# george-gca/sr-pytorch-lightning

Measured on AMD Instinct MI355X. Metric: SR training throughput, LR patches/s (48x48 LR x4, fwd+bwd+Adam), higher is better.
Workload: dtype bf16; 1 GPU; edsr_baseline x4, 48x48 LR patches, batch 256/GPU, train step (L1 + Adam); global_batch=256, parallelism=dp1, hip_graph=full

## Files before the change

### sr-pytorch-lightning_amd/csrc/hr_tail.hip

```cpp
#include "srk_common.h"

namespace {

SRK_DEV void sub_of(int a, int d, int& i, int& s) {
  const int ap = a + d;
  i = ap & 1;
  s = (ap - i) >> 1;
}

struct Wts {
  const float* wt; const float* bt; const float* wu; const float* bu;
  int O, C, Ci;
};

SRK_DEV float sum16(float v) {
  v += __shfl_xor(v, 8, 64);
  v += __shfl_xor(v, 4, 64);
  v += __shfl_xor(v, 2, 64);
  v += __shfl_xor(v, 1, 64);
  return v;
}

SRK_DEV float collapse_w(const Wts& p, int sub, int o, int a, int b, int ci, int dy0, int dy1, int dx0, int dx1, int fy, int fx) {
  float acc = 0.f;
// ... 216 lines not shown
  const bool shared_line = phase == 0 ? H == 1 : W == 1;
  if (shared_line && blockIdx.y == 1) return;
  extern __shared__ __attribute__((aligned(16))) char smem_raw[];
  const size_t gplane = (size_t)H2 * W2;
  const float* const g = a.g + (size_t)n * O * gplane;
  for (int rep = 0; rep < (shared_line ? 2 : 1); ++rep) {
  const EdgeGeo e = edge_geo(2 * phase + (shared_line ? rep : (int)blockIdx.y), H, W);
  float* const Gl = reinterpret_cast<float*>(smem_raw);
  float* const Wl = Gl + (size_t)2 * O * (e.len + 4);
  __syncthreads();
  for (int i0 = threadIdx.x; i0 < 2 * O * (e.len + 4); i0 += 256 * 4) {
    float v[4];
#pragma unroll
    for (int u = 0; u < 4; ++u) {
      const int i = i0 + 256 * u;
      const int kk = i / (e.len + 4), s = i % (e.len + 4) - 2, o = kk >> 1, q = kk & 1;
      v[u] = 0.f;
      if (i < 2 * O * (e.len + 4) && s >= 0 && s < e.len)
        v[u] = e.row ? g[(size_t)o * gplane + (size_t)e.fix_hr * W2 + 2 * s + q] : g[(size_t)o * gplane + (size_t)(2 * s + q) * W2 + e.fix_hr];
    }
#pragma unroll
    for (int u = 0; u < 4; ++u)
      if (i0 + 256 * u < 2 * O * (e.len + 4)) Gl[i0 + 256 * u] = v[u];
  }
  stage_copy256(Wl, a.wedge + (size_t)e.ty * 2 * O * Ci * 5, 2 * O * Ci * 5);
  __syncthreads();
  const int nch = (Ci + 7) >> 3;
  const bool vec = (Ci & 7) == 0 && (a.dx_pitch & 7) == 0;
  for (int idx = threadIdx.x + 256 * blockIdx.z; idx < e.len * nch; idx += 256 * gridDim.z) {
    const int c8 = idx % nch, s = idx / nch;
    float corr[8];
#pragma unroll
    for (int k = 0; k < 8; ++k) corr[k] = 0.f;
    for (int kk = 0; kk < 2 * O; ++kk) {
      const float* const gl = Gl + (size_t)kk * (e.len + 4) + s + 2;
      float gv[5];
#pragma unroll
      for (int tt = 0; tt < 5; ++tt) gv[tt] = gl[2 - tt];
#pragma unroll
      for (int k = 0; k < 8; ++k) {
        const int ci = c8 * 8 + k;
        if (ci < Ci) {
          const float* const w = Wl + ((size_t)kk * Ci + ci) * 5;
#pragma unroll
          for (int tt = 0; tt < 5; ++tt) corr[k] += w[tt] * gv[tt];
        }
      }
    }
    if (!e.row && (s == 0 || s == e.len - 1)) {
      for (int ca = 0; ca < 2; ++ca) {
        if (!(ca ? s == e.len - 1 : s == 0)) continue;
        const int cb = e.ty == 2 ? 0 : 1, c = ca * 2 + cb;
        const size_t at = (size_t)(ca ? H2 - 1 : 0) * W2 + e.fix_hr;
        for (int o = 0; o < O; ++o) {
          const float gc = g[(size_t)o * gplane + at];
#pragma unroll
          for (int k = 0; k < 8; ++k)
            if (c8 * 8 + k < Ci) corr[k] -= a.wcor[((size_t)c * O + o) * Ci + c8 * 8 + k] * gc;
        }
      }
    }
    const int yy = e.row ? e.fix_lr : s, xx = e.row ? s : e.fix_lr;
    typename Tr::elem* const d = reinterpret_cast<typename Tr::elem*>(a.dx) + ((size_t)(n * H + yy) * W + xx) * a.dx_pitch + c8 * 8;
    if (vec) {
      const i32x4 raw = *reinterpret_cast<const i32x4*>(d);
      const int w4[4] = {raw.x, raw.y, raw.z, raw.w};
      int o4[4];
#pragma unroll
      for (int k = 0; k < 4; ++k) {
        float f0, f1;
        unpack2<DT>((uint32_t)w4[k], f0, f1);
        o4[k] = (int)pack2<DT>(f0 - corr[2 * k], f1 - corr[2 * k + 1]);
      }
      *reinterpret_cast<i32x4*>(d) = i32x4{o4[0], o4[1], o4[2], o4[3]};
    } else {
#pragma unroll
      for (int k = 0; k < 8; ++k)
        if (c8 * 8 + k < Ci) d[k] = Tr::from_f32(Tr::to_f32(d[k]) - corr[k]);
    }
  }
  }
}

constexpr int EW_MAXLEN = 512;
template <int DT>
__global__ __launch_bounds__(256) void hrtail_edge_bwd_w_kernel(const srk_hrtail_args a, int nchunks, int ew_chunk) {
  const int H = a.H, W = a.W, O = a.O, Ci = a.Ci, H2 = 2 * H, W2 = 2 * W;
  const int ty = blockIdx.y, chunk = blockIdx.x;
  const int n0 = chunk * ew_chunk, n1 = min(a.N, n0 + ew_chunk);
  const int ncombo = ty < 4 ? 2 * O * 5 : O;
  const size_t gplane = (size_t)H2 * W2;
  float* const dst = a.scratch + ((size_t)ty * nchunks + chunk) * (size_t)(2 * MAXO * 5) * (Ci + 1);
  extern __shared__ __attribute__((aligned(16))) char smem_raw[];
  float* const Xl = reinterpret_cast<float*>(smem_raw);
  if (ty >= 4) {
    if (blockIdx.z != 0) return;
    const int c = ty - 4, ca = c >> 1, cbb = c & 1;
    const int Py = ca ? H2 - 1 : 0, Px = cbb ? W2 - 1 : 0, yy = ca ? H - 1 : 0, xx = cbb ? W - 1 : 0;
    for (int item = threadIdx.x; item < ncombo * (Ci + 1); item += 256) {
      const int ci = item % (Ci + 1), o = item / (Ci + 1);
      float acc = 0.f;
      for (int n = n0; n < n1; ++n) {
        const float gv = a.g[((size_t)n * O + o) * gplane + (size_t)Py * W2 + Px];
        const float xv = ci < Ci ? ld_act<DT>(a.x, ((size_t)(n * H + yy) * W + xx) * a.x_pitch + ci) : 1.f;
        acc += gv * xv;
      }
      dst[item] = acc;
    }
    return;
  }
  const bool rowedge = ty < 2;
  const int len = rowedge ? W : H;
  float* const Gl = Xl + (size_t)(len + 4) * Ci;
  constexpr int MAXIT = (2 * MAXO * 5 * 65 + 255) / 256;
  const int nitems = ncombo * (Ci + 1);
  const int ipb = (nitems + gridDim.z - 1) / gridDim.z, item0 = blockIdx.z * ipb, item1 = min(nitems, item0 + ipb);
  float acc[MAXIT];
#pragma unroll
  for (int k = 0; k < MAXIT; ++k) acc[k] = 0.f;
  for (int n = n0; n < n1; ++n) {
    __syncthreads();
    stage_line<DT>(a, edge_geo(ty, H, W), n, Xl, Ci);
    for (int i = threadIdx.x; i < 2 * O * len; i += 256) {
      const int kk = i / len, s = i % len, o = kk >> 1, q = kk & 1;
      const float* const g = a.g + ((size_t)n * O + o) * gplane;
      Gl[i] = rowedge ? g[(size_t)(ty == 0 ? 0 : H2 - 1) * W2 + 2 * s + q] : g[(size_t)(2 * s + q) * W2 + (ty == 2 ? 0 : W2 - 1)];
    }
    __syncthreads();
#pragma unroll
    for (int k = 0; k < MAXIT; ++k) {
      const int item = item0 + threadIdx.x + k * 256;
      if (item >= item1) break;
      const int ci = item % (Ci + 1), cb = item / (Ci + 1), tt = cb % 5, kk = cb / 5;
      const float* const gr = Gl + kk * len;
      float t0 = 0.f, t1 = 0.f, t2 = 0.f, t3 = 0.f;
      int p = 0;
      if (ci < Ci) {
        const float* const xr = Xl + (size_t)tt * Ci + ci;
        for (; p + 3 < len; p += 4) {
          t0 += gr[p] * xr[(size_t)p * Ci]; t1 += gr[p + 1] * xr[(size_t)(p + 1) * Ci];
          t2 += gr[p + 2] * xr[(size_t)(p + 2) * Ci]; t3 += gr[p + 3] * xr[(size_t)(p + 3) * Ci];
        }
        for (; p < len; ++p) t0 += gr[p] * xr[(size_t)p * Ci];
      } else if (tt == 2) {
        for (; p + 3 < len; p += 4) { t0 += gr[p]; t1 += gr[p + 1]; t2 += gr[p + 2]; t3 += gr[p + 3]; }
        for (; p < len; ++p) t0 += gr[p];
      }
      acc[k] += (t0 + t1) + (t2 + t3);
    }
  }
#pragma unroll
  for (int k = 0; k < MAXIT; ++k) {
    const int item = item0 + threadIdx.x + k * 256;
    if (item < item1) dst[item] = acc[k];
  }
}

__global__ __launch_bounds__(256) void hrtail_edge_reduce_kernel(const srk_hrtail_args a, int nchunks) {
  const int O = a.O, Ci = a.Ci;
  const int per = 2 * MAXO * 5 * (Ci + 1);
  const int t = blockIdx.x * 256 + threadIdx.x;
  const int n_edge = 4 * 2 * O * 5 * (Ci + 1), n_cor = 4 * O * (Ci + 1);
  if (t >= n_edge + n_cor) return;
  int ty, item;
  if (t < n_edge) { ty = t / (2 * O * 5 * (Ci + 1)); item = t % (2 * O * 5 * (Ci + 1)); }
  else { const int u = t - n_edge; ty = 4 + u / (O * (Ci + 1)); item = u % (O * (Ci + 1)); }
// ... 63 lines not shown
      }
    }
    acc = wave_total(acc);
    if (lane == 0) a.dwt[t] = acc;
    return;
  }
  int t = blockIdx.x * 256 + threadIdx.x;
  if (t < n_wu) {
    const int e = t % 9, ci = (t / 9) % Ci, cu = t / (9 * Ci), c = cu >> 2, i = (cu >> 1) & 1, j = cu & 1;
    const int ey = e / 3 - 1, ex = e % 3 - 1;
    float acc = 0.f;
    for (int pa = 0; pa < 2; ++pa)
      for (int dy = -1; dy <= 1; ++dy) {
        int ii, sy; sub_of(pa, dy, ii, sy);
        if (ii != i) continue;
        for (int pb = 0; pb < 2; ++pb)
          for (int dx = -1; dx <= 1; ++dx) {
            int jj, sx; sub_of(pb, dx, jj, sx);
            if (jj != j) continue;
            for (int o = 0; o < O; ++o)
              acc += a.wt[((size_t)o * C + c) * 9 + (dy + 1) * 3 + dx + 1] * g_w(q, o, pa, pb, dy, dx, ci, sy + ey, sx + ex);
          }
      }
    a.dwu[t] = acc;
    return;
  }
  t -= n_wu;
  if (t < n_bu) {
    if (!a.dbu) return;
    const int cu = t, c = cu >> 2, i = (cu >> 1) & 1, j = cu & 1;
    float acc = 0.f;
    for (int pa = 0; pa < 2; ++pa)
      for (int dy = -1; dy <= 1; ++dy) {
        int ii, sy; sub_of(pa, dy, ii, sy);
        if (ii != i) continue;
        for (int pb = 0; pb < 2; ++pb)
          for (int dx = -1; dx <= 1; ++dx) {
            int jj, sx; sub_of(pb, dx, jj, sx);
            if (jj != j) continue;
            for (int o = 0; o < O; ++o) acc += a.wt[((size_t)o * C + c) * 9 + (dy + 1) * 3 + dx + 1] * g_b(q, o, pa, pb, dy, dx);
          }
      }
    a.dbu[cu] = acc;
    return;
  }
  t -= n_bu;
  if (t < n_bt && a.dbt) a.dbt[t] = a.r0[t * 4] + a.r0[t * 4 + 1] + a.r0[t * 4 + 2] + a.r0[t * 4 + 3];
}

int check_common(const srk_hrtail_args* a, const char* who) {
  SRK_CHECK_ARG(a, "%s: null argument", who);
  SRK_CHECK_ARG(a->O >= 1 && a->O <= MAXO && a->C >= 1 && a->Ci >= 1, "%s: O=%d (1..%d) C=%d Ci=%d", who, a->O, MAXO, a->C, a->Ci);
  return 0;
}
int check_act(const srk_hrtail_args* a, const char* who) {
  SRK_CHECK_ARG(a->N > 0 && a->H > 0 && a->W > 0, "%s: bad dims N=%d H=%d W=%d", who, a->N, a->H, a->W);
  SRK_CHECK_ARG(a->dtype == SRK_BF16 || a->dtype == SRK_F16, "%s: 16-bit activations only", who);
  SRK_CHECK_ARG((long long)a->N * a->O * 4 * a->H * a->W < (1ll << 31), "%s: output too large", who);
  return 0;
}

}

extern "C" int srk_hrtail_collapse(const srk_hrtail_args* a, srk_stream_t stream) {
  if (int rc = check_common(a, "srk_hrtail_collapse")) return rc;
  SRK_CHECK_ARG(a->wt && a->wu && a->weff && a->beff && a->wedge && a->bedge && a->wcor && a->bcor, "srk_hrtail_collapse: null pointer");
  const int total = 4 * a->O * a->Ci * 25 + 4 * 2 * a->O * a->Ci * 5 + 4 * a->O * a->Ci + 16 * a->O;
  hipLaunchKernelGGL(hrtail_collapse_kernel, dim3((unsigned)((total + 15) / 16)), dim3(256), 0, reinterpret_cast<hipStream_t>(stream), *a);
  SRK_LAUNCH_CHECK();
  return 0;
}

static unsigned edge_split(int N) {
  const int z = (512 + 2 * N - 1) / (2 * N);
  return (unsigned)(z < 1 ? 1 : (z > 8 ? 8 : z));
}

template <typename K> static int edge_lds_attr(K kernel, const char* who) {
  const hipError_t e = hipFuncSetAttribute(reinterpret_cast<const void*>(kernel), hipFuncAttributeMaxDynamicSharedMemorySize, 160 * 1024);
  if (e != hipSuccess) { srk_set_error("%s: cannot reserve LDS: %s", who, hipGetErrorString(e)); return (int)e; }
  return 0;
}

extern "C" int srk_hrtail_edge_fwd(const srk_hrtail_args* a, srk_stream_t stream) {
  if (int rc = check_common(a, "srk_hrtail_edge_fwd")) return rc;
  if (int rc = check_act(a, "srk_hrtail_edge_fwd")) return rc;
  SRK_CHECK_ARG(a->x && a->out && a->wedge && a->bedge && a->wcor && a->bcor, "srk_hrtail_edge_fwd: null pointer");
  const int len = a->H > a->W ? a->H : a->W;
  const size_t lds = ((size_t)(len + 4) * (a->Ci + 1) + (size_t)2 * a->O * a->Ci * 5) * 4;
  SRK_CHECK_ARG(lds <= 160 * 1024, "srk_hrtail_edge_fwd: edge of %d pixels x %d channels does not fit the LDS", len, a->Ci);
  static const int rc0 = edge_lds_attr(&hrtail_edge_fwd_kernel<SRK_BF16>, "srk_hrtail_edge_fwd");
  static const int rc1 = edge_lds_attr(&hrtail_edge_fwd_kernel<SRK_F16>, "srk_hrtail_edge_fwd");
  if (rc0 || rc1) return rc0 ? rc0 : rc1;
  hipStream_t st = reinterpret_cast<hipStream_t>(stream);
  for (int phase = 0; phase < 2; ++phase) {
    if (a->dtype == SRK_BF16) hipLaunchKernelGGL(hrtail_edge_fwd_kernel<SRK_BF16>, dim3((unsigned)a->N, 2, edge_split(a->N)), dim3(256), lds, st, *a, phase);
    else hipLaunchKernelGGL(hrtail_edge_fwd_kernel<SRK_F16>, dim3((unsigned)a->N, 2, edge_split(a->N)), dim3(256), lds, st, *a, phase);
    SRK_LAUNCH_CHECK();
  }
  return 0;
}

extern "C" int srk_hrtail_edge_bwd_x(const srk_hrtail_args* a, srk_stream_t stream) {
  if (int rc = check_common(a, "srk_hrtail_edge_bwd_x")) return rc;
  if (int rc = check_act(a, "srk_hrtail_edge_bwd_x")) return rc;
  SRK_CHECK_ARG(a->g && a->dx && a->wedge && a->wcor, "srk_hrtail_edge_bwd_x: null pointer");
  const int len = a->H > a->W ? a->H : a->W;
  const size_t lds = ((size_t)2 * a->O * (len + 4) + (size_t)2 * a->O * a->Ci * 5) * 4;
  SRK_CHECK_ARG(lds <= 160 * 1024, "srk_hrtail_edge_bwd_x: edge of %d pixels does not fit the LDS", len);
  static const int rc0 = edge_lds_attr(&hrtail_edge_bwd_x_kernel<SRK_BF16>, "srk_hrtail_edge_bwd_x");
  static const int rc1 = edge_lds_attr(&hrtail_edge_bwd_x_kernel<SRK_F16>, "srk_hrtail_edge_bwd_x");
  if (rc0 || rc1) return rc0 ? rc0 : rc1;
  hipStream_t st = reinterpret_cast<hipStream_t>(stream);
  for (int phase = 0; phase < 2; ++phase) {
    if (a->dtype == SRK_BF16) hipLaunchKernelGGL(hrtail_edge_bwd_x_kernel<SRK_BF16>, dim3((unsigned)a->N, 2, edge_split(a->N)), dim3(256), lds, st, *a, phase);
    else hipLaunchKernelGGL(hrtail_edge_bwd_x_kernel<SRK_F16>, dim3((unsigned)a->N, 2, edge_split(a->N)), dim3(256), lds, st, *a, phase);
    SRK_LAUNCH_CHECK();
  }
  return 0;
}

static int ew_chunk_of(int N) { return N <= 64 ? 1 : (N + 63) / 64; }

extern "C" long long srk_hrtail_scratch_floats(int N, int Ci) {
  const int ewc = ew_chunk_of(N);
  const long long nchunks = (N + ewc - 1) / ewc;
  return 8 * nchunks * (long long)(2 * MAXO * 5) * (Ci + 1);
}

extern "C" int srk_hrtail_edge_bwd_w(const srk_hrtail_args* a, srk_stream_t stream) {
  if (int rc = check_common(a, "srk_hrtail_edge_bwd_w")) return rc;
  if (int rc = check_act(a, "srk_hrtail_edge_bwd_w")) return rc;
  SRK_CHECK_ARG(a->x && a->g && a->scratch && a->eedge && a->e0 && a->ecor && a->k0, "srk_hrtail_edge_bwd_w: null pointer");
  const int ewc = ew_chunk_of(a->N);
  const int nchunks = (a->N + ewc - 1) / ewc;
  const unsigned nz = nchunks * 8 >= 512 ? 2 : (nchunks * 8 >= 256 ? 4 : 8);
  const int len = a->H > a->W ? a->H : a->W;
  SRK_CHECK_ARG(a->Ci <= 64 && len <= EW_MAXLEN, "srk_hrtail_edge_bwd_w: Ci=%d (<= 64) edge length %d (<= %d)", a->Ci, len, EW_MAXLEN);
  const size_t lds = ((size_t)(len + 4) * a->Ci + (size_t)2 * a->O * len) * 4;
  hipStream_t st = reinterpret_cast<hipStream_t>(stream);
  static const hipError_t attr0 = hipFuncSetAttribute(reinterpret_cast<const void*>(&hrtail_edge_bwd_w_kernel<SRK_BF16>), hipFuncAttributeMaxDynamicSharedMemorySize, 160 * 1024);
  static const hipError_t attr1 = hipFuncSetAttribute(reinterpret_cast<const void*>(&hrtail_edge_bwd_w_kernel<SRK_F16>), hipFuncAttributeMaxDynamicSharedMemorySize, 160 * 1024);
  if (attr0 != hipSuccess || attr1 != hipSuccess) { srk_set_error("srk_hrtail_edge_bwd_w: cannot reserve LDS"); return (int)(attr0 != hipSuccess ? attr0 : attr1); }
  if (a->dtype == SRK_BF16) hipLaunchKernelGGL(hrtail_edge_bwd_w_kernel<SRK_BF16>, dim3((unsigned)nchunks, 8, nz), dim3(256), lds, st, *a, nchunks, ewc);
  else hipLaunchKernelGGL(hrtail_edge_bwd_w_kernel<SRK_F16>, dim3((unsigned)nchunks, 8, nz), dim3(256), lds, st, *a, nchunks, ewc);
  SRK_LAUNCH_CHECK();
  const int total = (4 * 2 * a->O * 5 + 4 * a->O) * (a->Ci + 1);
  hipLaunchKernelGGL(hrtail_edge_reduce_kernel, dim3((unsigned)((total + 255) / 256)), dim3(256), 0, st, *a, nchunks);
  SRK_LAUNCH_CHECK();
  return 0;
}

extern "C" int srk_hrtail_expand(const srk_hrtail_args* a, srk_stream_t stream) {
  if (int rc = check_common(a, "srk_hrtail_expand")) return rc;
  SRK_CHECK_ARG(a->wt && a->wu && a->r && a->r0 && a->eedge && a->e0 && a->ecor && a->k0 && a->dwt && a->dwu, "srk_hrtail_expand: null pointer");
  const int per_thread = 4 * a->C * a->Ci * 9 + 4 * a->C + a->O, per_wave = a->O * a->C * 9;
  const int nblocks = (per_thread + 255) / 256 + (per_wave + 3) / 4;
  hipLaunchKernelGGL(hrtail_expand_kernel, dim3((unsigned)nblocks), dim3(256), 0, reinterpret_cast<hipStream_t>(stream), *a);
  SRK_LAUNCH_CHECK();
  return 0;
}
```

### sr-pytorch-lightning_amd/csrc/conv_lk.hip

```cpp
#include <stdlib.h>
#include <type_traits>
#include "srk_common.h"

#ifndef SRK_LK5_STAMPS
#define SRK_LK5_STAMPS 0
#endif

namespace {

template <int DT, int CPP, int NRB, int K>
__global__ __launch_bounds__(256) void lk_conv_kernel(const srk_conv_args a, int tilesX, int tilesY, unsigned x_bytes, unsigned w_bytes) {
  typedef DTraits<DT> Tr;
  constexpr int PXB = CPP * 16;
  constexpr int ROWS = 32 * NRB;
  extern __shared__ __attribute__((aligned(16))) char smem[];
  constexpr int XT = 16 + K - 1, XTP = (XT + 1) & ~1;
  constexpr int xs_bytes = XT * XTP * PXB;
  constexpr int slab = K * CPP * ROWS * 16;
  char* const Xs = smem;
  char* const Wr = smem + ((xs_bytes + 1023) & ~1023);

  const int tid = threadIdx.x, lane = tid & 63;
  const int wave = __builtin_amdgcn_readfirstlane(tid >> 6);
  const int r = lane & 31, h = lane >> 5;
// ... 976 lines not shown
      if (lane < 8)
        dma16_hidden(xrsrc, (rok && (unsigned)(x0 + p1) < (unsigned)W) ? (unsigned)(base + c1) : 0x80000000u, (unsigned)__builtin_amdgcn_readfirstlane((int)(dst + 1024)));
    };
    asm volatile("s_waitcnt vmcnt(0) lgkmcnt(0)\n\ts_barrier" ::: "memory");
    dma_row(wave);
    dma_row(4 + wave);
    dma_row(8 + wave);
#if SRK_LK5_STAMPS
    unsigned long long* const stamp = (blockIdx.x == 0 && tid == 0 && u == blockIdx.x) ? reinterpret_cast<unsigned long long*>(const_cast<float*>(a.post_add)) : nullptr;
#define SRK_LSTAMP(i) do { if (stamp && s < 24) stamp[s * 8 + (i)] = __builtin_amdgcn_s_memtime(); } while (0)
#else
#define SRK_LSTAMP(i) do { } while (0)
#endif
    f32x16 accp[2];
    int gyp = 0;
    uint32_t P[4][4];
    auto epi_cvt = [&](int k) {
#pragma unroll
      for (int d = 0; d < 4; ++d) P[k][d] = pack2<DT>(accp[k >> 1][8 * (k & 1) + 2 * d], accp[k >> 1][8 * (k & 1) + 2 * d + 1]);
    };
    auto epi_store = [&](int j) {
      const int qi = r & 3, gxq = x0 + (r & ~3);
      const bool ok = gyp < ye && gxq + j < W;
      const unsigned off = (unsigned)((((n * H + gyp) * W + gxq + j) * a.out_pitch + a.out_coff + 32 * h + 8 * qi) * 2);
      const u32x4_t ov = {P[j][0], P[j][1], P[j][2], P[j][3]};
      __builtin_amdgcn_raw_buffer_store_b128(ov, orsrc, ok ? off : 0x80000000u, 0, SRK_AUX_WT);
    };
    auto step = [&](int s, auto epi_tag) {
      constexpr bool EPI = decltype(epi_tag)::value;
      SRK_LSTAMP(0);
      if (!EPI) asm volatile("s_waitcnt vmcnt(0)" ::: "memory");
      else if (s == 1) asm volatile("s_waitcnt vmcnt(2)" ::: "memory");
      else if (s == 2) asm volatile("s_waitcnt vmcnt(6)" ::: "memory");
      else asm volatile("s_waitcnt vmcnt(10)" ::: "memory");
      SRK_LSTAMP(1);
      asm volatile("s_waitcnt lgkmcnt(0)\n\ts_barrier" ::: "memory");
      SRK_LSTAMP(2);
      dma_row(4 * s + 12 + wave);
      const int q0 = 4 * s + wave;
      const char* rowp[5];
#pragma unroll
      for (int kh = 0; kh < 5; ++kh) rowp[kh] = smem + ((q0 + kh) % RING) * ROWB + r * 32 + h * 16;
      f32x16 acc[2];
#pragma unroll
      for (int e = 0; e < 16; ++e) { acc[0][e] = 0.f; acc[1][e] = 0.f; }
      constexpr int PF = 6;
      i32x4 bf[PF];
      auto bfrag = [&](int t) { return lds_read16(rowp[t / 5] + (t % 5) * 32); };
#pragma unroll
      for (int t = 0; t < PF; ++t) bf[t] = bfrag(t);
#pragma unroll
      for (int t = 0; t < 25; t += 2) {
        const i32x4 b0 = bf[t % PF], b1 = bf[(t + 1) % PF];
        if (t + PF < 25) bf[t % PF] = bfrag(t + PF);
        if (t + 1 + PF < 25) bf[(t + 1) % PF] = bfrag(t + 1 + PF);
        if (EPI) {
          if (t >= 2 && t < 10) epi_cvt((t - 2) >> 1);
          else if (t == 10) quad_transpose8_dpp(P[0][0], P[1][0], P[2][0], P[3][0], P[0][1], P[1][1], P[2][1], P[3][1]);
          else if (t == 12) quad_transpose8_dpp(P[0][2], P[1][2], P[2][2], P[3][2], P[0][3], P[1][3], P[2][3], P[3][3]);
          else if (t >= 14 && t < 22) epi_store((t - 14) >> 1);
        }
        acc[0] = Tr::mma(A[t][0], b0, acc[0]);
        if (t + 1 < 25) acc[0] = Tr::mma(A[t + 1][0], b1, acc[0]);
        acc[1] = Tr::mma(A[t][1], b0, acc[1]);
        if (t + 1 < 25) acc[1] = Tr::mma(A[t + 1][1], b1, acc[1]);
        __builtin_amdgcn_sched_barrier(0);
      }
      SRK_LSTAMP(3);
      accp[0] = acc[0]; accp[1] = acc[1];
      gyp = ys + q0;
    };
    step(0, std::false_type{});
#pragma unroll 1
    for (int s = 1; s < steps; ++s) step(s, std::true_type{});
#pragma unroll
    for (int k = 0; k < 4; ++k) epi_cvt(k);
    quad_transpose8_dpp(P[0][0], P[1][0], P[2][0], P[3][0], P[0][1], P[1][1], P[2][1], P[3][1]);
    quad_transpose8_dpp(P[0][2], P[1][2], P[2][2], P[3][2], P[0][3], P[1][3], P[2][3], P[3][3]);
#pragma unroll
    for (int j = 0; j < 4; ++j) epi_store(j);
  }
}

SRK_DEV void lk5_pair(int t, int& fyA, int& fxA, int& fyB, int& fxB, bool& hasB) {
  hasB = true;
  if (t < 5) { fyA = -2; fxA = t - 2; fyB = -1; fxB = t - 2; }
  else if (t < 10) { fyA = 0; fxA = t - 7; fyB = 1; fxB = t - 7; }
  else if (t == 10) { fyA = 2; fxA = -2; fyB = 2; fxB = 2; }
  else { fyA = 2; fxA = t - 12; fyB = 2; fxB = t - 12; hasB = false; }
}

template <int DT>
__global__ __launch_bounds__(256) void lk5_wgrad_kernel(const srk_wgrad_args a, int tilesX, int tilesY, int tq, int trem,
                                                        unsigned x_bytes, unsigned dy_bytes) {
  typedef DTraits<DT> Tr;
  constexpr int XB = 16 * 16 * 128, DP = 20, DB = 13 * 1024, BUF = XB + DB;
  extern __shared__ __attribute__((aligned(16))) char smem[];
  const int tid = threadIdx.x, lane = tid & 63;
  const int wave = __builtin_amdgcn_readfirstlane(tid >> 6);
  const int slot = blockIdx.x;
  const int H = a.H, W = a.W;
  const int t0 = slot * tq + min(slot, trem), nt = tq + (slot < trem ? 1 : 0);
  const i32x4 xrs = make_rsrc4(a.x, x_bytes), drs = make_rsrc4(a.dy, dy_bytes);
  const unsigned lds0 = lds_addr_of(smem);

  int xconst[8], xyx[8];
#pragma unroll
  for (int k = 0; k < 8; ++k) {
    const int i = tid + 256 * k, sl = i & 7, p = i >> 3, iy = p >> 4, ix = p & 15, c = sl ^ swz(ix);
    xconst[k] = ((iy * W + ix) * a.x_pitch + a.x_coff + c * 8) * 2;
    xyx[k] = iy | (ix << 8);
  }
  int dconst[4], dyx[4];
#pragma unroll
  for (int j = 0; j < 4; ++j) {
    const int i = tid + 256 * j, c = i & 1, pp = i >> 1, iy = pp / DP, ix = pp - iy * DP;
    dconst[j] = (((iy - 2) * W + (ix - 2)) * a.dy_pitch + a.dy_coff + c * 8) * 2;
    dyx[j] = i < 2 * DP * DP ? (((iy - 2) & 0xffff) | ((ix - 2) << 16)) : (int)0x7fff7fff;
  }
  auto dma_tile = [&](int tile, int b) {
    int pt = tile;
    const int tX = pt % tilesX;
    pt /= tilesX;
    const int tY = pt % tilesY;
    const int n = pt / tilesY;
    const int y0 = tY * 16, x0 = tX * 16;
    const int xbase = ((n * H + y0) * W + x0) * a.x_pitch * 2, dbase = ((n * H + y0) * W + x0) * a.dy_pitch * 2;
#pragma unroll
    for (int k = 0; k < 8; ++k) {
      const bool ok = y0 + (xyx[k] & 255) < H && x0 + (xyx[k] >> 8) < W;
      dma16_hidden(xrs, ok ? (unsigned)(xbase + xconst[k]) : 0x80000000u,
                   (unsigned)__builtin_amdgcn_readfirstlane((int)(lds0 + b * BUF + ((k * 256 + wave * 64) << 4))));
    }
#pragma unroll
    for (int j = 0; j < 4; ++j) {
      if (j * 256 + wave * 64 >= 2 * DP * DP) continue;
      const int gy = y0 + (int)(short)(dyx[j] & 0xffff), gx = x0 + (dyx[j] >> 16);
      const bool ok = (unsigned)gy < (unsigned)H && (unsigned)gx < (unsigned)W;
      dma16_hidden(drs, ok ? (unsigned)(dbase + dconst[j]) : 0x80000000u,
                   (unsigned)__builtin_amdgcn_readfirstlane((int)(lds0 + b * BUF + XB + ((j * 256 + wave * 64) << 4))));
    }
  };

  const int rb = wave & 1, half = wave >> 1;
  f32x16 acc[7];
#pragma unroll
  for (int j = 0; j < 7; ++j)
#pragma unroll
    for (int e = 0; e < 16; ++e) acc[j][e] = 0.f;
  int aoff[2], boff[7][2];
#pragma unroll
  for (int rd = 0; rd < 2; ++rd) aoff[rd] = tr_lane_off(0, rd, rb, lane);
  {
    const int G = lane >> 4, q = (lane & 15) >> 2, pq = lane & 3;
#pragma unroll
    for (int j = 0; j < 7; ++j) {
      int fyA, fxA, fyB, fxB; bool hasB;
      lk5_pair(half * 7 + j, fyA, fxA, fyB, fxB, hasB);
      const int fy = (G & 1) ? fyB : fyA, fx = (G & 1) ? fxB : fxA;
#pragma unroll
      for (int rd = 0; rd < 2; ++rd) {
        const int col = 8 * (G >> 1) + 4 * rd + q;
        boff[j][rd] = ((2 - fy) * DP + (col - fx + 2)) * 32 + pq * 8;
      }
    }
  }
  const bool do_bias = a.dbp != nullptr && wave == 2;
  float dbz = 0.f;

  const int pieces_of = 8 + (wave == 0 ? 4 : 3);
  if (nt > 0) dma_tile(t0, 0);
  if (nt > 1) dma_tile(t0 + 1, 1);
#if SRK_LK5_STAMPS
  unsigned long long* const wstamp = (blockIdx.x == 0 && tid == 0 && a.dbp) ? reinterpret_cast<unsigned long long*>(a.dbp) + (size_t)a.nslabs * 8 : nullptr;
#define SRK_WSTAMP(i) do { if (wstamp && it < 24) wstamp[it * 8 + (i)] = __builtin_amdgcn_s_memtime(); } while (0)
#else
#define SRK_WSTAMP(i) do { } while (0)
#endif
  for (int it = 0; it < nt; ++it) {
    SRK_WSTAMP(0);
    const char* const X = smem + (it % 3) * BUF;
    const char* const D = X + XB;
    if (it + 1 < nt) { if (pieces_of == 12) asm volatile("s_waitcnt vmcnt(12)" ::: "memory"); else asm volatile("s_waitcnt vmcnt(11)" ::: "memory"); }
    else asm volatile("s_waitcnt vmcnt(0)" ::: "memory");
    SRK_WSTAMP(1);
    asm volatile("s_waitcnt lgkmcnt(0)\n\ts_barrier" ::: "memory");
    SRK_WSTAMP(2);
    if (it + 2 < nt) dma_tile(t0 + it + 2, (it + 2) % 3);
    SRK_WSTAMP(3);
    i32x4 afn, bfn[7];
    auto fetch = [&](int y) {
      afn = tr_read2(X + y * 2048 + aoff[0], X + y * 2048 + aoff[1]);
#pragma unroll
      for (int j = 0; j < 7; ++j) bfn[j] = tr_read2(D + y * (DP * 32) + boff[j][0], D + y * (DP * 32) + boff[j][1]);
    };
    fetch(0);
#pragma unroll 2
    for (int y = 0; y < 16; ++y) {
      const i32x4 af = afn;
      i32x4 bf[7];
#pragma unroll
      for (int j = 0; j < 7; ++j) bf[j] = bfn[j];
      if (y + 1 < 16) fetch(y + 1);
      if (do_bias) {
        const int qw[4] = {bf[0].x, bf[0].y, bf[0].z, bf[0].w};
#pragma unroll
        for (int e = 0; e < 4; ++e) {
          float f0, f1;
          unpack2<DT>((uint32_t)qw[e], f0, f1);
          dbz += f0 + f1;
        }
      }
#pragma unroll
      for (int j = 0; j < 7; ++j) acc[j] = Tr::mma(af, bf[j], acc[j]);
    }
    SRK_WSTAMP(4);
  }

  if (do_bias) {
    dbz += __shfl_xor(dbz, 32, 64);
    if (lane < 16) a.dbp[(size_t)slot * 16 + lane] = dbz;
  }
  {
    const int hq = lane >> 5, n = lane & 31, co = n & 15;
    float* const sl = a.dwp + (size_t)slot * (25 * 64 * 16);
#pragma unroll
    for (int j = 0; j < 7; ++j) {
      int fyA, fxA, fyB, fxB; bool hasB;
      lk5_pair(half * 7 + j, fyA, fxA, fyB, fxB, hasB);
      if (n >= 16 && !hasB) continue;
      const int tap = n < 16 ? (fyA + 2) * 5 + fxA + 2 : (fyB + 2) * 5 + fxB + 2;
#pragma unroll
      for (int e = 0; e < 16; ++e) {
        const int ci = rb * 32 + 4 * hq + (e & 3) + 8 * (e >> 2);
        sl[((size_t)tap * 64 + ci) * 16 + co] = acc[j][e];
      }
    }
  }
}

bool lk5_wgrad_ok(const srk_wgrad_args& a) {
  static const bool off = [] { const char* e = srk_dbg_getenv("SRK_NO_LK5"); return e && e[0] == '1'; }();
  return !off && a.KH == 5 && a.Cin == 64 && a.Cout == 16 && (a.cout_real == 0 || a.cout_real > 6) && a.x_pitch % 8 == 0 && a.dy_pitch % 8 == 0 &&
         a.x_coff % 8 == 0 && a.dy_coff % 8 == 0;
}

bool lk_all_rows(const srk_wgrad_args& a) {
  static const bool off = [] { const char* e = srk_dbg_getenv("SRK_NO_LK_ALLROWS"); const char* p = srk_dbg_getenv("SRK_NO_LK_PACKED"); return (e && e[0] == '1') || (p && p[0] == '1'); }();
  return !off && a.cout_real > 0 && a.cout_real <= LK_CS && a.cout_real * a.KW <= 32 && a.KH >= 5;
}

int lk_wgrad_slabs_for(const srk_wgrad_args& a) {
  static const int cus = [] { int c = srk_device_cus(); return c > 0 ? c : 256; }();
  if (lk_all_rows(a)) {
    const long long nt8 = (long long)a.N * ((a.H + LK_TR - 1) / LK_TR) * ((a.W + 15) / 16);
    return (int)(nt8 < cus ? nt8 : cus);
  }
  const long long ntiles = (long long)a.N * ((a.H + 15) / 16) * ((a.W + 15) / 16);
  if (lk5_wgrad_ok(a)) return (int)(ntiles < cus ? ntiles : cus);
  long long s = cus / a.KH;
  if (s < 1) s = 1;
  if (s > ntiles) s = ntiles;
  return (int)s;
}

}

bool srk_conv_lk_ok(const srk_conv_args& a) {
  if (a.dtype == SRK_F32 || a.KH != a.KW || a.KH < 5 || a.KH > 9 || !(a.KH & 1)) return false;
  if (a.x_ps > 1 || a.mask) return false;
  const bool fwd = a.Cin == 64 && a.CoutP == 32;
  const bool bwd = a.Cin == 16 && a.CoutP == 64;
  if (!fwd && !bwd) return false;
  if (a.out_mode == SRK_OUT_PLANAR) {
    if (!fwd || a.ps_r != 2 || a.res || a.relu || a.Cout % 4 || a.Cout > 16 || a.x_pitch % 8 || a.x_coff % 8) return false;
    return (long long)a.N * a.H * a.W * a.x_pitch * 2 < 0x7fff0000LL;
  }
  if (a.out_mode != SRK_OUT_NHWC || (a.post_add && !SRK_LK5_STAMPS)) return false;
  if (a.x_pitch % 8 || a.x_coff % 8 || a.out_pitch % 8 || a.out_coff % 8 || a.Cout % 8 || (a.res && (a.res_pitch % 8 || a.res_coff % 8))) return false;
  const long long px = (long long)a.N * a.H * a.W;
  long long mx = px * a.x_pitch;
  if (px * a.out_pitch > mx) mx = px * a.out_pitch;
  return mx * 2 < 0x7fff0000LL;
}

template <int DT, int CPP, int NRB, int K> static int lk_launch_k(const srk_conv_args& a, hipStream_t st) {
  constexpr int XT = 16 + K - 1, XTP = (XT + 1) & ~1;
  constexpr int xs = (XT * XTP * CPP * 16 + 1023) & ~1023, slab = K * CPP * 32 * NRB * 16;
  constexpr int lds = xs + 2 * slab;
  static const hipError_t attr = hipFuncSetAttribute(reinterpret_cast<const void*>(&lk_conv_kernel<DT, CPP, NRB, K>),
                                                     hipFuncAttributeMaxDynamicSharedMemorySize, 160 * 1024);
  if (attr != hipSuccess) { srk_set_error("srk_conv2d: cannot reserve LDS for the large-kernel conv"); return (int)attr; }
  SRK_CHECK_ARG(lds <= 160 * 1024, "srk_conv2d: %dx%d kernel needs %d bytes of LDS", K, K, lds);
  const int tilesX = (a.W + 15) / 16, tilesY = (a.H + 15) / 16;
  const long long nb = (long long)a.N * tilesX * tilesY;
  SRK_CHECK_ARG(nb <= 0x7fffffffLL, "srk_conv2d: %lld workgroups", nb);
  hipLaunchKernelGGL((lk_conv_kernel<DT, CPP, NRB, K>), dim3((unsigned)nb), dim3(256), lds, st, a, tilesX, tilesY,
                     (unsigned)((long long)a.N * a.H * a.W * a.x_pitch * 2), (unsigned)((long long)K * slab));
  SRK_LAUNCH_CHECK();
  return 0;
}
template <int DT, int CPP, int NRB> static int lk_launch(const srk_conv_args& a, hipStream_t st) {
  switch (a.KH) {
    case 5: return lk_launch_k<DT, CPP, NRB, 5>(a, st);
    case 7: return lk_launch_k<DT, CPP, NRB, 7>(a, st);
    default: return lk_launch_k<DT, CPP, NRB, 9>(a, st);
  }
}

template <int DT, int K> static int lk_rows_launch_k(const srk_conv_args& a, hipStream_t st) {
  constexpr int XWP = (16 + K - 1 + 1) & ~1, XR = 8 + K - 1;
  constexpr int lds = ((XR * XWP * 128 + 1023) & ~1023) + 4 * 4096 + 4 * 512;
// ... 159 lines not shown
```

Measured before the change: 47660 LR patches/s.

## Add MFMA paths for HR-tail edge forward and input-gradient kernels

Adds matrix-core (MFMA) versions of the edge forward and edge input-backward kernels for the HR tail when Ci is 64 and the data is aligned. Work is split into 32-pixel runs per wave. The fp32 weights are split into several bf16/f16 parts so the matrix products keep near-fp32 accuracy. These kernels replace the scalar LDS-heavy kernels that used large dynamic LDS and one block per image. The cost is a more complex precision-splitting scheme, and the border pixels only touch a small fraction of the image, so the effect on the full step is limited.

```diff
diff --git a/sr-pytorch-lightning_amd/csrc/hr_tail.hip b/sr-pytorch-lightning_amd/csrc/hr_tail.hip
--- a/sr-pytorch-lightning_amd/csrc/hr_tail.hip
+++ b/sr-pytorch-lightning_amd/csrc/hr_tail.hip
@@ -322,6 +322,229 @@
   }
 }
 
+constexpr int ER = 32;
+constexpr int ERP = ER + 4;
+constexpr int EDGE_W_FLOATS = 2 * MAXO * 64 * 5;
+SRK_DEV int eoff(int li, int c) { return (li << 7) + ((c ^ swz(li)) << 4); }
+template <int DT> SRK_DEV float round16(float f) { return DTraits<DT>::to_f32(DTraits<DT>::from_f32(f)); }
+template <int DT> SRK_DEV float split3(float w, int part) {
+  constexpr float SC = DT == SRK_F16 ? 2048.f : 1.f;
+  const float p0 = round16<DT>(w);
+  const float r1 = (w - p0) * SC, p1 = round16<DT>(r1);
+  const float r2 = (r1 - p1) * SC, p2 = round16<DT>(r2);
+  return part == 0 ? p0 : (part == 1 ? p1 : p2);
+}
+SRK_DEV void wave_lds_fence() {
+  __builtin_amdgcn_fence(__ATOMIC_ACQ_REL, "wavefront");
+  __builtin_amdgcn_wave_barrier();
+}
+
+template <int DT>
+__global__ __launch_bounds__(256) void hrtail_edge_fwd_mfma_kernel(const srk_hrtail_args a, int phase) {
+  typedef DTraits<DT> Tr;
+  constexpr float ISC = DT == SRK_F16 ? 1.f / 2048.f : 1.f;
+  const int H = a.H, W = a.W, O = a.O, H2 = 2 * H, W2 = 2 * W;
+  const EdgeGeo e = edge_geo(2 * phase + blockIdx.y, H, W);
+  const int lane = threadIdx.x & 63, wave = threadIdx.x >> 6;
+  __shared__ __attribute__((aligned(16))) char smem[EDGE_W_FLOATS * 4 + 4 * ERP * 128];
+  float* const Wl = reinterpret_cast<float*>(smem);
+  char* const img = smem + EDGE_W_FLOATS * 4 + wave * (ERP * 128);
+  stage_copy256(Wl, a.wedge + (size_t)e.ty * 2 * O * 64 * 5, 2 * O * 64 * 5);
+  __syncthreads();
+  const int r = lane & 31, h = lane >> 5;
+  i32x4 A[20];
+  {
+    const int part = r >> 3, kk = r & 7;
+    const bool live = part < 3 && kk < 2 * O;
+#pragma unroll
+    for (int ks = 0; ks < 20; ++ks) {
+      const int tt = ks >> 2, ci0 = (ks & 3) * 16 + 8 * h;
+      int pk[4];
+#pragma unroll
+      for (int j = 0; j < 4; ++j) {
+        const float w0 = live ? Wl[(kk * 64 + ci0 + 2 * j) * 5 + tt] : 0.f, w1 = live ? Wl[(kk * 64 + ci0 + 2 * j + 1) * 5 + tt] : 0.f;
+        pk[j] = (int)pack2<DT>(split3<DT>(w0, part), split3<DT>(w1, part));
+      }
+      A[ks] = i32x4{pk[0], pk[1], pk[2], pk[3]};
+    }
+  }
+  float be[4];
+#pragma unroll
+  for (int q = 0; q < 4; ++q) be[q] = 4 * h + q < 2 * O ? a.bedge[e.ty * 2 * O + 4 * h + q] : 0.f;
+  const int runs = (e.len + ER - 1) / ER, nitems = a.N * runs;
+  const size_t oplane = (size_t)H2 * W2;
+  for (int item = blockIdx.x * 4 + wave; item < nitems; item += gridDim.x * 4) {
+    const int n = item / runs, s0 = (item - n * runs) * ER;
+    wave_lds_fence();
+    {
+      i32x4 raw[5];
+#pragma unroll
+      for (int u = 0; u < 5; ++u) {
+        const int i = lane + 64 * u, li = i >> 3, c = i & 7, s = s0 - 2 + li;
+        raw[u] = i32x4{0, 0, 0, 0};
+        if (i < ERP * 8 && s >= 0 && s < e.len) {
+          const int yy = e.row ? e.fix_lr : s, xx = e.row ? s : e.fix_lr;
+          raw[u] = gload16(reinterpret_cast<const typename Tr::elem*>(a.x) + ((size_t)(n * H + yy) * W + xx) * a.x_pitch + c * 8);
+        }
+      }
+#pragma unroll
+      for (int u = 0; u < 5; ++u) {
+        const int i = lane + 64 * u;
+        if (i < ERP * 8) lds_write16(img + eoff(i >> 3, i & 7), raw[u]);
+      }
+    }
+    wave_lds_fence();
+    f32x16 acc;
+#pragma unroll
+    for (int k = 0; k < 16; ++k) acc[k] = 0.f;
+#pragma unroll
+    for (int ks = 0; ks < 20; ++ks) acc = Tr::mma(A[ks], lds_read16(img + eoff(r + (ks >> 2), (ks & 3) * 2 + h)), acc);
+    float cc[2][MAXO];
+#pragma unroll
+    for (int ca = 0; ca < 2; ++ca)
+#pragma unroll
+      for (int o = 0; o < MAXO; ++o) cc[ca][o] = 0.f;
+    if (!e.row) {
+#pragma unroll
+      for (int ca = 0; ca < 2; ++ca) {
+        const int sc = ca ? e.len - 1 : 0;
+        if (sc < s0 || sc >= s0 + ER) continue;
+        const int c = ca * 2 + (e.ty == 2 ? 0 : 1), li = sc - s0 + 2;
+        const float xv = Tr::to_f32(*reinterpret_cast<const typename Tr::elem*>(img + eoff(li, lane >> 3) + (lane & 7) * 2));
+#pragma unroll
+        for (int o = 0; o < MAXO; ++o)
+          if (o < O) cc[ca][o] = a.bcor[c * O + o] + wave_sum64(a.wcor[((size_t)c * O + o) * 64 + lane] * xv);
+      }
+    }
+    const int s = s0 + r;
+    if (s < e.len) {
+      float* const out = a.out + (size_t)n * O * oplane;
+#pragma unroll
+      for (int q4 = 0; q4 < 4; ++q4) {
+        const int kk = 4 * h + q4, o = kk >> 1, q = kk & 1, p = 2 * s + q;
+        if (kk >= 2 * O) continue;
+        float v = be[q4] + (acc[q4] + (acc[q4 + 4] + acc[q4 + 8] * ISC) * ISC);
+        if (!e.row) {
+          const float c0 = h ? cc[0][2 + (q4 >> 1)] : cc[0][q4 >> 1], c1 = h ? cc[1][2 + (q4 >> 1)] : cc[1][q4 >> 1];
+          if (p == 0) v -= c0;
+          else if (p == 2 * e.len - 1) v -= c1;
+        }
+        const size_t at = e.row ? (size_t)e.fix_hr * W2 + p : (size_t)p * W2 + e.fix_hr;
+        out[(size_t)o * oplane + at] -= v;
+      }
+    }
+  }
+}
+
+template <int DT>
+__global__ __launch_bounds__(256) void hrtail_edge_bwd_x_mfma_kernel(const srk_hrtail_args a, int phase) {
+  typedef DTraits<DT> Tr;
+  typedef DTraits<SRK_BF16> Bf;
+  const int H = a.H, W = a.W, O = a.O, H2 = 2 * H, W2 = 2 * W;
+  const EdgeGeo e = edge_geo(2 * phase + blockIdx.y, H, W);
+  const int lane = threadIdx.x & 63, wave = threadIdx.x >> 6;
+  __shared__ __attribute__((aligned(16))) char smem[EDGE_W_FLOATS * 4 + 4 * 2 * ERP * 16];
+  float* const Wl = reinterpret_cast<float*>(smem);
+  char* const Gh = smem + EDGE_W_FLOATS * 4 + wave * (2 * ERP * 16);
+  char* const Gl = Gh + ERP * 16;
+  stage_copy256(Wl, a.wedge + (size_t)e.ty * 2 * O * 64 * 5, 2 * O * 64 * 5);
+  __syncthreads();
+  const int col = lane & 15, g4 = lane >> 4;
+  i32x4 A[4][4];
+#pragma unroll
+  for (int mt = 0; mt < 4; ++mt) {
+    const int ci = (col >> 2) * 16 + mt * 4 + (col & 3);
+#pragma unroll
+    for (int ks = 0; ks < 4; ++ks) {
+      const int m = ks * 4 + g4, term = m / 5, tt = m - term * 5;
+      float v[8];
+#pragma unroll
+      for (int j = 0; j < 8; ++j) {
+        const float w = (m < 15 && j < 2 * O) ? Wl[(j * 64 + ci) * 5 + tt] : 0.f;
+        const float hi = round16<SRK_BF16>(w);
+        v[j] = term == 1 ? round16<SRK_BF16>(w - hi) : hi;
+      }
+      A[mt][ks] = i32x4{(int)pack2<SRK_BF16>(v[0], v[1]), (int)pack2<SRK_BF16>(v[2], v[3]), (int)pack2<SRK_BF16>(v[4], v[5]), (int)pack2<SRK_BF16>(v[6], v[7])};
+    }
+  }
+  int boff[4];
+#pragma unroll
+  for (int ks = 0; ks < 4; ++ks) {
+    const int m = min(ks * 4 + g4, 14), term = m / 5, tt = m - term * 5;
+    boff[ks] = (term == 2 ? ERP * 16 : 0) + (col + 4 - tt) * 16;
+  }
+  const int runs = (e.len + ER - 1) / ER, nitems = a.N * runs;
+  const size_t gplane = (size_t)H2 * W2;
+  for (int item = blockIdx.x * 4 + wave; item < nitems; item += gridDim.x * 4) {
+    const int n = item / runs, s0 = (item - n * runs) * ER;
+    const float* const g = a.g + (size_t)n * O * gplane;
+    wave_lds_fence();
+    {
+      float v[5];
+#pragma unroll
+      for (int u = 0; u < 5; ++u) {
+        const int i = lane + 64 * u, o = i / (2 * ERP), pp = i - o * (2 * ERP), li = pp >> 1, q = pp & 1, s = s0 - 2 + li;
+        v[u] = 0.f;
+        if (i < 8 * ERP && o < O && s >= 0 && s < e.len)
+          v[u] = e.row ? g[(size_t)o * gplane + (size_t)e.fix_hr * W2 + 2 * s + q] : g[(size_t)o * gplane + (size_t)(2 * s + q) * W2 + e.fix_hr];
+      }
+#pragma unroll
+      for (int u = 0; u < 5; ++u) {
+        const int i = lane + 64 * u, o = i / (2 * ERP), pp = i - o * (2 * ERP), li = pp >> 1, q = pp & 1;
+        if (i >= 8 * ERP) continue;
+        const uint16_t hi = Bf::from_f32(v[u]);
+        *reinterpret_cast<uint16_t*>(Gh + li * 16 + (o * 2 + q) * 2) = hi;
+        *reinterpret_cast<uint16_t*>(Gl + li * 16 + (o * 2 + q) * 2) = Bf::from_f32(v[u] - Bf::to_f32(hi));
+      }
+    }
+    wave_lds_fence();
+#pragma unroll
+    for (int nt = 0; nt < 2; ++nt) {
+      f32x4 acc[4];
+#pragma unroll
+      for (int mt = 0; mt < 4; ++mt) acc[mt] = f32x4{0.f, 0.f, 0.f, 0.f};
+#pragma unroll
+      for (int ks = 0; ks < 4; ++ks) {
+        const bf16x8 b = __builtin_bit_cast(bf16x8, lds_read16(Gh + boff[ks] + nt * 16 * 16));
+#pragma unroll
+        for (int mt = 0; mt < 4; ++mt) acc[mt] = __builtin_amdgcn_mfma_f32_16x16x32_bf16(__builtin_bit_cast(bf16x8, A[mt][ks]), b, acc[mt], 0, 0, 0);
+      }
+      const int s = s0 + nt * 16 + col;
+      if (s >= e.len) continue;
+      float corr[16];
+#pragma unroll
+      for (int k = 0; k < 16; ++k) corr[k] = acc[k >> 2][k & 3];
+      if (!e.row && (s == 0 || s == e.len - 1)) {
+        for (int ca = 0; ca < 2; ++ca) {
+          if (!(ca ? s == e.len - 1 : s == 0)) continue;
+          const int cb = e.ty == 2 ? 0 : 1, c = ca * 2 + cb;
+          const size_t at = (size_t)(ca ? H2 - 1 : 0) * W2 + e.fix_hr;
+          for (int o = 0; o < O; ++o) {
+            const float gc = g[(size_t)o * gplane + at];
+#pragma unroll
+            for (int k = 0; k < 16; ++k) corr[k] -= a.wcor[((size_t)c * O + o) * 64 + g4 * 16 + k] * gc;
+          }
+        }
+      }
+      const int yy = e.row ? e.fix_lr : s, xx = e.row ? s : e.fix_lr;
+      typename Tr::elem* const d = reinterpret_cast<typename Tr::elem*>(a.dx) + ((size_t)(n * H + yy) * W + xx) * a.dx_pitch + g4 * 16;
+#pragma unroll
+      for (int half = 0; half < 2; ++half) {
+        const i32x4 raw = *reinterpret_cast<const i32x4*>(d + half * 8);
+        const int w4[4] = {raw.x, raw.y, raw.z, raw.w};
+        int o4[4];
+#pragma unroll
+        for (int k = 0; k < 4; ++k) {
+          float f0, f1;
+          unpack2<DT>((uint32_t)w4[k], f0, f1);
+          o4[k] = (int)pack2<DT>(f0 - corr[half * 8 + 2 * k], f1 - corr[half * 8 + 2 * k + 1]);
+        }
+        *reinterpret_cast<i32x4*>(d + half * 8) = i32x4{o4[0], o4[1], o4[2], o4[3]};
+      }
+    }
+  }
+}
+
 constexpr int EW_MAXLEN = 512;
 template <int DT>
 __global__ __launch_bounds__(256) void hrtail_edge_bwd_w_kernel(const srk_hrtail_args a, int nchunks, int ew_chunk) {
@@ -551,17 +774,38 @@
   return 0;
 }
 
+static bool edge_scalar_forced() {
+  const char* e = srk_dbg_getenv("SRK_HRTAIL_EDGE_SCALAR");
+  return e && e[0] == '1';
+}
+static bool edge_mfma_ok(const srk_hrtail_args* a, const void* act, int pitch) {
+  return a->Ci == 64 && (pitch & 7) == 0 && ((uintptr_t)act & 15) == 0 && !edge_scalar_forced();
+}
+static unsigned edge_mfma_wgs(int N, int len) {
+  const long long items = (long long)N * ((len + ER - 1) / ER);
+  return (unsigned)((items + 3) / 4 > 1024 ? 1024 : (items + 3) / 4);
+}
+
 extern "C" int srk_hrtail_edge_fwd(const srk_hrtail_args* a, srk_stream_t stream) {
   if (int rc = check_common(a, "srk_hrtail_edge_fwd")) return rc;
   if (int rc = check_act(a, "srk_hrtail_edge_fwd")) return rc;
   SRK_CHECK_ARG(a->x && a->out && a->wedge && a->bedge && a->wcor && a->bcor, "srk_hrtail_edge_fwd: null pointer");
+  hipStream_t st = reinterpret_cast<hipStream_t>(stream);
+  if (edge_mfma_ok(a, a->x, a->x_pitch)) {
+    for (int phase = 0; phase < 2; ++phase) {
+      const dim3 grid(edge_mfma_wgs(a->N, phase ? a->H : a->W), 2);
+      if (a->dtype == SRK_BF16) hipLaunchKernelGGL(hrtail_edge_fwd_mfma_kernel<SRK_BF16>, grid, dim3(256), 0, st, *a, phase);
+      else hipLaunchKernelGGL(hrtail_edge_fwd_mfma_kernel<SRK_F16>, grid, dim3(256), 0, st, *a, phase);
+      SRK_LAUNCH_CHECK();
+    }
+    return 0;
+  }
   const int len = a->H > a->W ? a->H : a->W;
   const size_t lds = ((size_t)(len + 4) * (a->Ci + 1) + (size_t)2 * a->O * a->Ci * 5) * 4;
   SRK_CHECK_ARG(lds <= 160 * 1024, "srk_hrtail_edge_fwd: edge of %d pixels x %d channels does not fit the LDS", len, a->Ci);
   static const int rc0 = edge_lds_attr(&hrtail_edge_fwd_kernel<SRK_BF16>, "srk_hrtail_edge_fwd");
   static const int rc1 = edge_lds_attr(&hrtail_edge_fwd_kernel<SRK_F16>, "srk_hrtail_edge_fwd");
   if (rc0 || rc1) return rc0 ? rc0 : rc1;
-  hipStream_t st = reinterpret_cast<hipStream_t>(stream);
   for (int phase = 0; phase < 2; ++phase) {
     if (a->dtype == SRK_BF16) hipLaunchKernelGGL(hrtail_edge_fwd_kernel<SRK_BF16>, dim3((unsigned)a->N, 2, edge_split(a->N)), dim3(256), lds, st, *a, phase);
     else hipLaunchKernelGGL(hrtail_edge_fwd_kernel<SRK_F16>, dim3((unsigned)a->N, 2, edge_split(a->N)), dim3(256), lds, st, *a, phase);
@@ -581,8 +825,14 @@
   static const int rc1 = edge_lds_attr(&hrtail_edge_bwd_x_kernel<SRK_F16>, "srk_hrtail_edge_bwd_x");
   if (rc0 || rc1) return rc0 ? rc0 : rc1;
   hipStream_t st = reinterpret_cast<hipStream_t>(stream);
+  const bool mfma = edge_mfma_ok(a, a->dx, a->dx_pitch);
   for (int phase = 0; phase < 2; ++phase) {
-    if (a->dtype == SRK_BF16) hipLaunchKernelGGL(hrtail_edge_bwd_x_kernel<SRK_BF16>, dim3((unsigned)a->N, 2, edge_split(a->N)), dim3(256), lds, st, *a, phase);
+    const bool shared_line = phase == 0 ? a->H == 1 : a->W == 1;
+    if (mfma && !shared_line) {
+      const dim3 grid(edge_mfma_wgs(a->N, phase ? a->H : a->W), 2);
+      if (a->dtype == SRK_BF16) hipLaunchKernelGGL(hrtail_edge_bwd_x_mfma_kernel<SRK_BF16>, grid, dim3(256), 0, st, *a, phase);
+      else hipLaunchKernelGGL(hrtail_edge_bwd_x_mfma_kernel<SRK_F16>, grid, dim3(256), 0, st, *a, phase);
+    } else if (a->dtype == SRK_BF16) hipLaunchKernelGGL(hrtail_edge_bwd_x_kernel<SRK_BF16>, dim3((unsigned)a->N, 2, edge_split(a->N)), dim3(256), lds, st, *a, phase);
     else hipLaunchKernelGGL(hrtail_edge_bwd_x_kernel<SRK_F16>, dim3((unsigned)a->N, 2, edge_split(a->N)), dim3(256), lds, st, *a, phase);
     SRK_LAUNCH_CHECK();
   }
```

After: 47760 LR patches/s, median of 4. No clear change (+0.2%).

## Reuse dy LDS fragments across vertical taps in 5x5 wgrad kernel

Applied to the files above, without the earlier changes.

Regroups the 25 filter taps of the 5x5 weight-gradient kernel into three column streams per wave half. Each tap tile becomes a row-lagged view of a stream, so one LDS transpose read per stream and row is shared by several MFMA tiles, replacing seven reads per row. The cost is a large register array (3x20 fragments), full unrolling of the 16-row loop and a sched_barrier per row, which may raise register pressure and limit scheduling freedom.

```diff
diff --git a/sr-pytorch-lightning_amd/csrc/conv_lk.hip b/sr-pytorch-lightning_amd/csrc/conv_lk.hip
--- a/sr-pytorch-lightning_amd/csrc/conv_lk.hip
+++ b/sr-pytorch-lightning_amd/csrc/conv_lk.hip
@@ -1082,12 +1082,19 @@
   }
 }
 
-SRK_DEV void lk5_pair(int t, int& fyA, int& fxA, int& fyB, int& fxB, bool& hasB) {
-  hasB = true;
-  if (t < 5) { fyA = -2; fxA = t - 2; fyB = -1; fxB = t - 2; }
-  else if (t < 10) { fyA = 0; fxA = t - 7; fyB = 1; fxB = t - 7; }
-  else if (t == 10) { fyA = 2; fxA = -2; fyB = 2; fxB = 2; }
-  else { fyA = 2; fxA = t - 12; fyB = 2; fxB = t - 12; hasB = false; }
+SRK_DEV void lk5_stream(int half, int s, int& fyA, int& fxA, int& fyB, int& fxB) {
+  if (half == 1 && s == 2) { fyA = 2; fxA = -2; fyB = 2; fxB = 2; return; }
+  const int fx = half == 0 ? (s == 0 ? -2 : s == 1 ? 2 : -1) : s;
+  fyA = -2; fxA = fx; fyB = -1; fxB = fx;
+}
+constexpr int lk5_tile_stream(int half, int j) { return half == 0 ? (j < 2 ? 0 : j < 4 ? 1 : 2) : (j < 3 ? 0 : j < 6 ? 1 : 2); }
+constexpr int lk5_tile_lag(int half, int j) { return half == 0 ? (j < 4 ? 2 * (j & 1) : 2 * (j - 4)) : (j < 6 ? 2 * (j % 3) : 0); }
+constexpr int lk5_stream_depth(int half, int s) { return half == 0 ? (s == 2 ? 4 : 2) : (s == 2 ? 0 : 4); }
+SRK_DEV void lk5_tile(int half, int j, int& fyA, int& fxA, int& fyB, int& fxB, bool& hasB) {
+  lk5_stream(half, lk5_tile_stream(half, j), fyA, fxA, fyB, fxB);
+  fyA += lk5_tile_lag(half, j);
+  fyB += lk5_tile_lag(half, j);
+  hasB = fyB <= 2;
 }
 
 template <int DT>
@@ -1148,20 +1155,21 @@
   for (int j = 0; j < 7; ++j)
 #pragma unroll
     for (int e = 0; e < 16; ++e) acc[j][e] = 0.f;
-  int aoff[2], boff[7][2];
+  int aoff[2], boff[3][2], boff0[3][2];
 #pragma unroll
   for (int rd = 0; rd < 2; ++rd) aoff[rd] = tr_lane_off(0, rd, rb, lane);
   {
     const int G = lane >> 4, q = (lane & 15) >> 2, pq = lane & 3;
 #pragma unroll
-    for (int j = 0; j < 7; ++j) {
-      int fyA, fxA, fyB, fxB; bool hasB;
-      lk5_pair(half * 7 + j, fyA, fxA, fyB, fxB, hasB);
+    for (int s = 0; s < 3; ++s) {
+      int fyA, fxA, fyB, fxB;
+      lk5_stream(half, s, fyA, fxA, fyB, fxB);
       const int fy = (G & 1) ? fyB : fyA, fx = (G & 1) ? fxB : fxA;
 #pragma unroll
       for (int rd = 0; rd < 2; ++rd) {
         const int col = 8 * (G >> 1) + 4 * rd + q;
-        boff[j][rd] = ((2 - fy) * DP + (col - fx + 2)) * 32 + pq * 8;
+        boff[s][rd] = ((2 - fy) * DP + (col - fx + 2)) * 32 + pq * 8;
+        boff0[s][rd] = ((2 - fyA) * DP + (col - fx + 2)) * 32 + pq * 8;
       }
     }
   }
@@ -1188,32 +1196,48 @@
     SRK_WSTAMP(2);
     if (it + 2 < nt) dma_tile(t0 + it + 2, (it + 2) % 3);
     SRK_WSTAMP(3);
-    i32x4 afn, bfn[7];
-    auto fetch = [&](int y) {
-      afn = tr_read2(X + y * 2048 + aoff[0], X + y * 2048 + aoff[1]);
-#pragma unroll
-      for (int j = 0; j < 7; ++j) bfn[j] = tr_read2(D + y * (DP * 32) + boff[j][0], D + y * (DP * 32) + boff[j][1]);
+    auto tile = [&](auto half_tag) {
+      constexpr int HALF = decltype(half_tag)::value;
+      i32x4 R[3][20], afn;
+      auto rd = [&](int s, int y) { return tr_read2(D + y * (DP * 32) + boff[s][0], D + y * (DP * 32) + boff[s][1]); };
+#pragma unroll
+      for (int s = 0; s < 3; ++s) {
+        if (lk5_stream_depth(HALF, s) == 4) {
+          R[s][0] = tr_read2(D - 4 * (DP * 32) + boff0[s][0], D - 4 * (DP * 32) + boff0[s][1]);
+          R[s][1] = rd(s, -3);
+        }
+        if (lk5_stream_depth(HALF, s) >= 2) {
+          R[s][2] = rd(s, -2);
+          R[s][3] = rd(s, -1);
+        }
+        R[s][4] = rd(s, 0);
+      }
+      afn = tr_read2(X + aoff[0], X + aoff[1]);
+#pragma unroll
+      for (int y = 0; y < 16; ++y) {
+        const i32x4 af = afn;
+        if (y + 1 < 16) {
+          afn = tr_read2(X + (y + 1) * 2048 + aoff[0], X + (y + 1) * 2048 + aoff[1]);
+#pragma unroll
+          for (int s = 0; s < 3; ++s) R[s][y + 5] = rd(s, y + 1);
+        }
+        if (HALF == 1 && do_bias) {
+          const i32x4 b = R[0][y + 2];
+          const int qw[4] = {b.x, b.y, b.z, b.w};
+#pragma unroll
+          for (int e = 0; e < 4; ++e) {
+            float f0, f1;
+            unpack2<DT>((uint32_t)qw[e], f0, f1);
+            dbz += f0 + f1;
+          }
+        }
+#pragma unroll
+        for (int j = 0; j < 7; ++j) acc[j] = Tr::mma(af, R[lk5_tile_stream(HALF, j)][y + 4 - lk5_tile_lag(HALF, j)], acc[j]);
+        __builtin_amdgcn_sched_barrier(0);
+      }
     };
-    fetch(0);
-#pragma unroll 2
-    for (int y = 0; y < 16; ++y) {
-      const i32x4 af = afn;
-      i32x4 bf[7];
-#pragma unroll
-      for (int j = 0; j < 7; ++j) bf[j] = bfn[j];
-      if (y + 1 < 16) fetch(y + 1);
-      if (do_bias) {
-        const int qw[4] = {bf[0].x, bf[0].y, bf[0].z, bf[0].w};
-#pragma unroll
-        for (int e = 0; e < 4; ++e) {
-          float f0, f1;
-          unpack2<DT>((uint32_t)qw[e], f0, f1);
-          dbz += f0 + f1;
-        }
-      }
-#pragma unroll
-      for (int j = 0; j < 7; ++j) acc[j] = Tr::mma(af, bf[j], acc[j]);
-    }
+    if (half == 0) tile(std::integral_constant<int, 0>{});
+    else tile(std::integral_constant<int, 1>{});
     SRK_WSTAMP(4);
   }
 
@@ -1227,7 +1251,7 @@
 #pragma unroll
     for (int j = 0; j < 7; ++j) {
       int fyA, fxA, fyB, fxB; bool hasB;
-      lk5_pair(half * 7 + j, fyA, fxA, fyB, fxB, hasB);
+      lk5_tile(half, j, fyA, fxA, fyB, fxB, hasB);
       if (n >= 16 && !hasB) continue;
       const int tap = n < 16 ? (fyA + 2) * 5 + fxA + 2 : (fyB + 2) * 5 + fxB + 2;
 #pragma unroll
```

After: 47370 LR patches/s before, 47360 LR patches/s after, median of 2. About the same (-0.0%).
